# friendlymatthew/heif

Hardware: NVIDIA B200
Metric: decoded MP/s (12MP HEIC grid batch) (higher is better)
Workload: dtype u8

## Files before the change

heif_b200/csrc/cuda/deblock_kernel.cu:

```cuda
#include <cuda_runtime.h>

#include "kernels.h"

namespace heic {
namespace dev {

namespace {

__device__ const uint8_t kBetaTable[52] = {0,  0,  0,  0,  0,  0,  0,  0,  0,  0,  0,  0,  0,  0,  0,  0,  6,  7,
                                           8,  9,  10, 11, 12, 13, 14, 15, 16, 17, 18, 20, 22, 24, 26, 28, 30, 32,
                                           34, 36, 38, 40, 42, 44, 46, 48, 50, 52, 54, 56, 58, 60, 62, 64};
__device__ const uint8_t kTcTable[54] = {0, 0, 0, 0, 0, 0, 0, 0, 0, 0, 0,  0,  0,  0,  0,  0,  0,  0,
                                         1, 1, 1, 1, 1, 1, 1, 1, 1, 2, 2,  2,  2,  3,  3,  3,  3,  4,
                                         4, 4, 5, 5, 6, 6, 7, 8, 9, 10, 11, 13, 14, 16, 18, 20, 22, 24};
__device__ const uint8_t kChromaQp[14] = {29, 30, 31, 32, 33, 33, 34, 34, 35, 35, 36, 36, 37, 37};

__device__ __forceinline__ int clip3(int lo, int hi, int v) { return min(hi, max(lo, v)); }
__device__ __forceinline__ int clip8(int v) { return min(255, max(0, v)); }

__device__ __forceinline__ uint32_t interleave4(uint32_t v) {
  v &= 0x0fu;
  v = (v | (v << 2)) & 0x33u;
  v = (v | (v << 1)) & 0x55u;
  return v;
}

struct Pic {
  const uint32_t* tu_map;
  const uint8_t* qp_map;
  int w8, log2_ctb, wctb;
};

__device__ __forceinline__ bool is_tu_edge(const Pic& p, int x, int y, int pos) {
  const int ctb4 = 1 << (p.log2_ctb - 2);
  const int rx = x >> p.log2_ctb, ry = y >> p.log2_ctb;
  const uint32_t z = interleave4((uint32_t)(x >> 2) & (ctb4 - 1)) | (interleave4((uint32_t)(y >> 2) & (ctb4 - 1)) << 1);
  const uint32_t* tu = p.tu_map + (size_t)(ry * p.wctb + rx) * (ctb4 * ctb4);
  const uint32_t w3 = tu[z & ~63u], w2 = tu[z & ~15u];
  const bool in32 = (w3 & 7u) == (TU_ORIGIN | (3u << 1)) && (pos & 31) != 0;
  const bool in16 = (w2 & 7u) == (TU_ORIGIN | (2u << 1)) && (pos & 15) != 0;
  return !(in32 || in16);
}
__device__ __forceinline__ int qp_at(const Pic& p, int x, int y) { return p.qp_map[(y >> 3) * p.w8 + (x >> 3)]; }

__device__ __forceinline__ int dp4(uint32_t samples, uint32_t weights, int acc) {
  int d;
  asm("dp4a.u32.s32 %0, %1, %2, %3;" : "=r"(d) : "r"(samples), "r"(weights), "r"(acc));
  return d;
}
__host__ __device__ constexpr uint32_t W(int a, int b, int c, int d) {
  return ((uint32_t)a & 0xffu) | (((uint32_t)b & 0xffu) << 8) | (((uint32_t)c & 0xffu) << 16) | (((uint32_t)d & 0xffu) << 24);
}
__device__ __forceinline__ int lin(uint32_t P, uint32_t Q, uint32_t wp, uint32_t wq, int c) { return dp4(Q, wq, dp4(P, wp, c)); }

__device__ __forceinline__ bool filter_luma_segment(uint32_t (&rw)[8][2], int qp_sum, int beta_off2, int tc_off2) {
  const int qpl = (qp_sum + 1) >> 1;
  const int beta = kBetaTable[clip3(0, 51, qpl + beta_off2)];
  const int tc = kTcTable[clip3(0, 53, qpl + 2 + tc_off2)];
  const uint32_t P0 = rw[0][0], Q0 = rw[0][1], P3 = rw[3][0], Q3 = rw[3][1];
  const int dp0 = abs(dp4(P0, W(0, 1, -2, 1), 0)), dp3 = abs(dp4(P3, W(0, 1, -2, 1), 0));
  const int dq0 = abs(dp4(Q0, W(1, -2, 1, 0), 0)), dq3 = abs(dp4(Q3, W(1, -2, 1, 0), 0));
  const int dpq0 = dp0 + dq0, dpq3 = dp3 + dq3, dp = dp0 + dp3, dq = dq0 + dq3;
  if (dpq0 + dpq3 >= beta) return false;
  const int tc25 = (5 * tc + 1) >> 1;
  const bool s0 = 2 * dpq0 < (beta >> 2) && abs(dp4(P0, W(1, 0, 0, -1), 0)) + abs(dp4(Q0, W(1, 0, 0, -1), 0)) < (beta >> 3) &&
                  abs(lin(P0, Q0, W(0, 0, 0, 1), W(-1, 0, 0, 0), 0)) < tc25;
  const bool s3 = 2 * dpq3 < (beta >> 2) && abs(dp4(P3, W(1, 0, 0, -1), 0)) + abs(dp4(Q3, W(1, 0, 0, -1), 0)) < (beta >> 3) &&
                  abs(lin(P3, Q3, W(0, 0, 0, 1), W(-1, 0, 0, 0), 0)) < tc25;
  const bool strong = s0 && s3;
  const bool dep = dp < ((beta + (beta >> 1)) >> 3), deq = dq < ((beta + (beta >> 1)) >> 3);
#pragma unroll
  for (int l = 0; l < 4; l++) {
    const uint32_t P = rw[l][0], Q = rw[l][1];
    if (strong) {
      const int t2 = 2 * tc;
      const int e_p0 = clip3(-t2, t2, lin(P, Q, W(0, 1, 2, 2 - 8), W(2, 1, 0, 0), 4) >> 3);
      const int e_p1 = clip3(-t2, t2, lin(P, Q, W(0, 1, 1 - 4, 1), W(1, 0, 0, 0), 2) >> 2);
      const int e_p2 = clip3(-t2, t2, lin(P, Q, W(2, 3 - 8, 1, 1), W(1, 0, 0, 0), 4) >> 3);
      const int e_q0 = clip3(-t2, t2, lin(P, Q, W(0, 0, 1, 2), W(2 - 8, 2, 1, 0), 4) >> 3);
      const int e_q1 = clip3(-t2, t2, lin(P, Q, W(0, 0, 0, 1), W(1, 1 - 4, 1, 0), 2) >> 2);
      const int e_q2 = clip3(-t2, t2, lin(P, Q, W(0, 0, 0, 1), W(1, 1, 3 - 8, 2), 4) >> 3);
      rw[l][0] = P + (uint32_t)e_p2 * 256u + (uint32_t)e_p1 * 65536u + (uint32_t)e_p0 * 16777216u;
      rw[l][1] = Q + (uint32_t)e_q0 + (uint32_t)e_q1 * 256u + (uint32_t)e_q2 * 65536u;
    } else {
      int delta = lin(P, Q, W(0, 0, 3, -9), W(9, -3, 0, 0), 8) >> 4;
      if (abs(delta) < tc * 10) {
        delta = clip3(-tc, tc, delta);
        const int p0 = dp4(P, W(0, 0, 0, 1), 0), q0 = dp4(Q, W(1, 0, 0, 0), 0);
        const int ep = clip8(p0 + delta) - p0, eq = clip8(q0 - delta) - q0;
        uint32_t addp = (uint32_t)ep * 16777216u, addq = (uint32_t)eq;
        if (dep) {
          const int p1 = dp4(P, W(0, 0, 1, 0), 0);
          const int e = clip3(-(tc >> 1), tc >> 1, (((dp4(P, W(0, 1, 0, 1), 1) >> 1) - p1 + delta) >> 1));
          addp += (uint32_t)(clip8(p1 + e) - p1) * 65536u;
        }
        if (deq) {
          const int q1 = dp4(Q, W(0, 1, 0, 0), 0);
          const int e = clip3(-(tc >> 1), tc >> 1, (((dp4(Q, W(1, 0, 1, 0), 1) >> 1) - q1 - delta) >> 1));
          addq += (uint32_t)(clip8(q1 + e) - q1) * 256u;
        }
        rw[l][0] = P + addp;
        rw[l][1] = Q + addq;
      }
    }
  }
  return true;
}

__device__ __forceinline__ bool filter_chroma_segment(uint32_t (&rw)[8][2], int qp_sum, int c_qp_off, int tc_off2) {
  const int qpi = ((qp_sum + 1) >> 1) + c_qp_off;
  const int qpc = qpi < 30 ? qpi : (qpi >= 43 ? qpi - 6 : kChromaQp[qpi - 30]);
  const int tc = kTcTable[clip3(0, 53, qpc + 2 + tc_off2)];
  if (!tc) return false;
#pragma unroll
  for (int l = 0; l < 4; l++) {
    const uint32_t P = rw[l][0], Q = rw[l][1];
    const int delta = clip3(-tc, tc, lin(P, Q, W(0, 0, 1, -4), W(4, -1, 0, 0), 4) >> 3);
    const int p0 = dp4(P, W(0, 0, 0, 1), 0), q0 = dp4(Q, W(1, 0, 0, 0), 0);
    rw[l][0] = P + (uint32_t)(clip8(p0 + delta) - p0) * 16777216u;
    rw[l][1] = Q + (uint32_t)(clip8(q0 - delta) - q0);
  }
  return true;
}

__device__ __forceinline__ void transpose4(uint32_t a, uint32_t b, uint32_t c, uint32_t d, uint32_t& o0, uint32_t& o1, uint32_t& o2, uint32_t& o3) {
  const uint32_t t0 = __byte_perm(a, b, 0x5140), t1 = __byte_perm(c, d, 0x5140);
  const uint32_t t2 = __byte_perm(a, b, 0x7362), t3 = __byte_perm(c, d, 0x7362);
  o0 = __byte_perm(t0, t1, 0x5410);
  o1 = __byte_perm(t0, t1, 0x7632);
  o2 = __byte_perm(t2, t3, 0x5410);
  o3 = __byte_perm(t2, t3, 0x7632);
}
__device__ __forceinline__ void transpose_cell(uint32_t (&rw)[8][2]) {
  uint32_t t[8][2];
  transpose4(rw[0][0], rw[1][0], rw[2][0], rw[3][0], t[0][0], t[1][0], t[2][0], t[3][0]);
  transpose4(rw[4][0], rw[5][0], rw[6][0], rw[7][0], t[0][1], t[1][1], t[2][1], t[3][1]);
  transpose4(rw[0][1], rw[1][1], rw[2][1], rw[3][1], t[4][0], t[5][0], t[6][0], t[7][0]);
  transpose4(rw[4][1], rw[5][1], rw[6][1], rw[7][1], t[4][1], t[5][1], t[6][1], t[7][1]);
#pragma unroll
  for (int r = 0; r < 8; r++) rw[r][0] = t[r][0], rw[r][1] = t[r][1];
}

template <int CIDX>
__device__ __forceinline__ void deblock_cell(const Pic& pic, uint8_t* plane, int pitch, int pw, int ph, int k, int j,
                                             int beta_off2, int tc_off2, int c_qp_off) {
  constexpr int SUB = CIDX ? 1 : 0;
  const int x0 = 8 * k - 4, y0 = 8 * j - 4;
  const bool has_left = k > 0, has_right = 8 * k < pw, has_top = j > 0, has_bottom = 8 * j < ph;
  uint32_t rw[8][2];
#pragma unroll
  for (int r = 0; r < 8; r++) {
    const bool row_ok = r < 4 ? has_top : has_bottom;
    rw[r][0] = rw[r][1] = 0;
    if (row_ok) {
      const uint8_t* row = plane + (size_t)(y0 + r) * pitch;
      if (has_left) rw[r][0] = *reinterpret_cast<const uint32_t*>(row + x0);
      if (has_right) rw[r][1] = *reinterpret_cast<const uint32_t*>(row + x0 + 4);
    }
  }
  const int xe = (8 * k) << SUB, ye = (8 * j) << SUB;
  uint32_t seg_do = 0, seg_qp = 0;
#pragma unroll
  for (int g = 0; g < 4; g++) {
    const bool vert = g < 2;
    const int half = g & 1;
    bool ok;
    if (vert) ok = has_left && has_right && (half == 0 ? has_top : has_bottom);
    else ok = has_top && has_bottom && (half == 0 ? has_left : has_right);
    if (ok) {
      const int xl = vert ? xe : (x0 + 4 * half) << SUB, yl = vert ? (y0 + 4 * half) << SUB : ye;
      seg_qp |= (uint32_t)(qp_at(pic, xl, yl) + (vert ? qp_at(pic, xl - 1, yl) : qp_at(pic, xl, yl - 1))) << (8 * g);
      seg_do |= (is_tu_edge(pic, xl, yl, vert ? xl : yl) ? 1u : 0u) << g;
    }
  }
  if (!seg_do) return;
  bool changed = false;
#pragma unroll 1
  for (int g = 0; g < 4; g++) {
    if ((seg_do >> g) & 1u) {
      const int qp_sum = (int)((seg_qp >> (8 * g)) & 0xffu);
      changed |= CIDX == 0 ? filter_luma_segment(rw, qp_sum, beta_off2, tc_off2) : filter_chroma_segment(rw, qp_sum, c_qp_off, tc_off2);
    }
#pragma unroll
    for (int r = 0; r < 4; r++) {
      uint32_t t0 = rw[r][0], t1 = rw[r][1];
      rw[r][0] = rw[r + 4][0], rw[r][1] = rw[r + 4][1];
      rw[r + 4][0] = t0, rw[r + 4][1] = t1;
    }
    if (g & 1) transpose_cell(rw);
  }
  if (!changed) return;
#pragma unroll
  for (int r = 0; r < 8; r++) {
    const bool row_ok = r < 4 ? has_top : has_bottom;
    if (!row_ok) continue;
    uint8_t* row = plane + (size_t)(y0 + r) * pitch;
    if (has_left) *reinterpret_cast<uint32_t*>(row + x0) = rw[r][0];
    if (has_right) *reinterpret_cast<uint32_t*>(row + x0 + 4) = rw[r][1];
  }
}

#ifndef HEIC_DEBLOCK_MIN_CTAS
#define HEIC_DEBLOCK_MIN_CTAS 12
#endif
template <int KIND>
__global__ void __launch_bounds__(128, HEIC_DEBLOCK_MIN_CTAS) deblock_kernel(Arenas A, uint32_t blocks_per_tile) {
  const uint32_t tile = blockIdx.x / blocks_per_tile;
  const TileParams* tp = A.tiles + tile;
  const PicParams* pp = A.pics + tp->pic;
  if (A.status[tile].code != 0 || tp->deblock_disabled) return;
  if (KIND == 1 && !pp->chroma) return;
  uint32_t g = (blockIdx.x % blocks_per_tile) * blockDim.x + threadIdx.x;
  const int pw = pp->w >> KIND, ph = pp->h >> KIND;
  const uint32_t cx = (uint32_t)((pw + 7) >> 3) + 1, cy = (uint32_t)((ph + 7) >> 3) + 1;
  int cidx = KIND;
  if (g >= cx * cy) {
    if (KIND == 0) return;
    g -= cx * cy;
    cidx = 2;
    if (g >= cx * cy) return;
  }
  const int k = (int)(g % cx), j = (int)(g / cx);
  if (8 * k - 4 >= pw || 8 * j - 4 >= ph) return;
  Pic pic;
  pic.tu_map = A.tu_map + tp->tu_off;
  pic.qp_map = A.qp_map + tp->map8_off;
  pic.w8 = pp->w8;
  pic.log2_ctb = pp->log2_ctb;
  pic.wctb = pp->wctb;
  const int beta_off2 = tp->beta_offset_div2 * 2, tc_off2 = tp->tc_offset_div2 * 2;
  deblock_cell<KIND>(pic, A.recon + tp->plane_off[cidx], KIND ? pp->pitch_c : pp->pitch_y, pw, ph, k, j, beta_off2, tc_off2,
                     cidx == 0 ? 0 : (cidx == 1 ? pp->pps_cb_qp_offset : pp->pps_cr_qp_offset));
}

}

cudaError_t launch_deblock(const Arenas& A, uint32_t max_w, uint32_t max_h, cudaStream_t stream) {
  if (!A.n_tiles) return cudaSuccess;
  const uint32_t cells_y = (((max_w + 7) >> 3) + 1) * (((max_h + 7) >> 3) + 1);
  const uint32_t cells_c = 2 * ((((max_w >> 1) + 7) >> 3) + 1) * ((((max_h >> 1) + 7) >> 3) + 1);
  const uint32_t by = (cells_y + 127) / 128, bc = (cells_c + 127) / 128;
  deblock_kernel<0><<<A.n_tiles * by, 128, 0, stream>>>(A, by);
  deblock_kernel<1><<<A.n_tiles * bc, 128, 0, stream>>>(A, bc);
  return cudaGetLastError();
}

}
}
```

Measured before the change: 29020.

## Warp-compact luma deblock filtering by strong/normal class through shared staging

Splits the luma segment filter into a decision step and per-line filters. Each segment's lines are staged in shared memory and redistributed across the warp: strong-filter lines are processed first, then normal-filter lines, one line per lane. The aim is to cut divergence between strong and normal paths across lanes. The change also hoists the QP and TU-map lookups so shared corner values are loaded once per cell, and keeps out-of-range luma threads alive so warp ballots stay full. In exchange it adds shared-memory traffic, __syncwarp barriers and ballot overhead for every segment, plus extra work on dead lanes.

```diff
diff --git a/heif_b200/csrc/cuda/deblock_kernel.cu b/heif_b200/csrc/cuda/deblock_kernel.cu
--- a/heif_b200/csrc/cuda/deblock_kernel.cu
+++ b/heif_b200/csrc/cuda/deblock_kernel.cu
@@ -31,15 +31,16 @@
   int w8, log2_ctb, wctb;
 };
 
-__device__ __forceinline__ bool is_tu_edge(const Pic& p, int x, int y, int pos) {
+__device__ __forceinline__ uint32_t tu_units(const Pic& p, int x, int y) {
   const int ctb4 = 1 << (p.log2_ctb - 2);
   const int rx = x >> p.log2_ctb, ry = y >> p.log2_ctb;
   const uint32_t z = interleave4((uint32_t)(x >> 2) & (ctb4 - 1)) | (interleave4((uint32_t)(y >> 2) & (ctb4 - 1)) << 1);
   const uint32_t* tu = p.tu_map + (size_t)(ry * p.wctb + rx) * (ctb4 * ctb4);
   const uint32_t w3 = tu[z & ~63u], w2 = tu[z & ~15u];
-  const bool in32 = (w3 & 7u) == (TU_ORIGIN | (3u << 1)) && (pos & 31) != 0;
-  const bool in16 = (w2 & 7u) == (TU_ORIGIN | (2u << 1)) && (pos & 15) != 0;
-  return !(in32 || in16);
+  return (uint32_t)((w3 & 7u) == (TU_ORIGIN | (3u << 1))) | (uint32_t)((w2 & 7u) == (TU_ORIGIN | (2u << 1))) << 1;
+}
+__device__ __forceinline__ uint32_t is_tu_edge(uint32_t units, int pos) {
+  return !(((units & 1u) && (pos & 31) != 0) || ((units & 2u) && (pos & 15) != 0));
 }
 __device__ __forceinline__ int qp_at(const Pic& p, int x, int y) { return p.qp_map[(y >> 3) * p.w8 + (x >> 3)]; }
 
@@ -53,7 +54,7 @@
 }
 __device__ __forceinline__ int lin(uint32_t P, uint32_t Q, uint32_t wp, uint32_t wq, int c) { return dp4(Q, wq, dp4(P, wp, c)); }
 
-__device__ __forceinline__ bool filter_luma_segment(uint32_t (&rw)[8][2], int qp_sum, int beta_off2, int tc_off2) {
+__device__ __forceinline__ uint32_t decide_luma_segment(const uint32_t (&rw)[8][2], int qp_sum, int beta_off2, int tc_off2) {
   const int qpl = (qp_sum + 1) >> 1;
   const int beta = kBetaTable[clip3(0, 51, qpl + beta_off2)];
   const int tc = kTcTable[clip3(0, 53, qpl + 2 + tc_off2)];
@@ -61,50 +62,84 @@
   const int dp0 = abs(dp4(P0, W(0, 1, -2, 1), 0)), dp3 = abs(dp4(P3, W(0, 1, -2, 1), 0));
   const int dq0 = abs(dp4(Q0, W(1, -2, 1, 0), 0)), dq3 = abs(dp4(Q3, W(1, -2, 1, 0), 0));
   const int dpq0 = dp0 + dq0, dpq3 = dp3 + dq3, dp = dp0 + dp3, dq = dq0 + dq3;
-  if (dpq0 + dpq3 >= beta) return false;
   const int tc25 = (5 * tc + 1) >> 1;
-  const bool s0 = 2 * dpq0 < (beta >> 2) && abs(dp4(P0, W(1, 0, 0, -1), 0)) + abs(dp4(Q0, W(1, 0, 0, -1), 0)) < (beta >> 3) &&
-                  abs(lin(P0, Q0, W(0, 0, 0, 1), W(-1, 0, 0, 0), 0)) < tc25;
-  const bool s3 = 2 * dpq3 < (beta >> 2) && abs(dp4(P3, W(1, 0, 0, -1), 0)) + abs(dp4(Q3, W(1, 0, 0, -1), 0)) < (beta >> 3) &&
-                  abs(lin(P3, Q3, W(0, 0, 0, 1), W(-1, 0, 0, 0), 0)) < tc25;
-  const bool strong = s0 && s3;
+  const bool s0 = (2 * dpq0 < (beta >> 2)) & (abs(dp4(P0, W(1, 0, 0, -1), 0)) + abs(dp4(Q0, W(1, 0, 0, -1), 0)) < (beta >> 3)) &
+                  (abs(lin(P0, Q0, W(0, 0, 0, 1), W(-1, 0, 0, 0), 0)) < tc25);
+  const bool s3 = (2 * dpq3 < (beta >> 2)) & (abs(dp4(P3, W(1, 0, 0, -1), 0)) + abs(dp4(Q3, W(1, 0, 0, -1), 0)) < (beta >> 3)) &
+                  (abs(lin(P3, Q3, W(0, 0, 0, 1), W(-1, 0, 0, 0), 0)) < tc25);
   const bool dep = dp < ((beta + (beta >> 1)) >> 3), deq = dq < ((beta + (beta >> 1)) >> 3);
-#pragma unroll
-  for (int l = 0; l < 4; l++) {
-    const uint32_t P = rw[l][0], Q = rw[l][1];
-    if (strong) {
-      const int t2 = 2 * tc;
-      const int e_p0 = clip3(-t2, t2, lin(P, Q, W(0, 1, 2, 2 - 8), W(2, 1, 0, 0), 4) >> 3);
-      const int e_p1 = clip3(-t2, t2, lin(P, Q, W(0, 1, 1 - 4, 1), W(1, 0, 0, 0), 2) >> 2);
-      const int e_p2 = clip3(-t2, t2, lin(P, Q, W(2, 3 - 8, 1, 1), W(1, 0, 0, 0), 4) >> 3);
-      const int e_q0 = clip3(-t2, t2, lin(P, Q, W(0, 0, 1, 2), W(2 - 8, 2, 1, 0), 4) >> 3);
-      const int e_q1 = clip3(-t2, t2, lin(P, Q, W(0, 0, 0, 1), W(1, 1 - 4, 1, 0), 2) >> 2);
-      const int e_q2 = clip3(-t2, t2, lin(P, Q, W(0, 0, 0, 1), W(1, 1, 3 - 8, 2), 4) >> 3);
-      rw[l][0] = P + (uint32_t)e_p2 * 256u + (uint32_t)e_p1 * 65536u + (uint32_t)e_p0 * 16777216u;
-      rw[l][1] = Q + (uint32_t)e_q0 + (uint32_t)e_q1 * 256u + (uint32_t)e_q2 * 65536u;
-    } else {
-      int delta = lin(P, Q, W(0, 0, 3, -9), W(9, -3, 0, 0), 8) >> 4;
-      if (abs(delta) < tc * 10) {
-        delta = clip3(-tc, tc, delta);
-        const int p0 = dp4(P, W(0, 0, 0, 1), 0), q0 = dp4(Q, W(1, 0, 0, 0), 0);
-        const int ep = clip8(p0 + delta) - p0, eq = clip8(q0 - delta) - q0;
-        uint32_t addp = (uint32_t)ep * 16777216u, addq = (uint32_t)eq;
-        if (dep) {
-          const int p1 = dp4(P, W(0, 0, 1, 0), 0);
-          const int e = clip3(-(tc >> 1), tc >> 1, (((dp4(P, W(0, 1, 0, 1), 1) >> 1) - p1 + delta) >> 1));
-          addp += (uint32_t)(clip8(p1 + e) - p1) * 65536u;
-        }
-        if (deq) {
-          const int q1 = dp4(Q, W(0, 1, 0, 0), 0);
-          const int e = clip3(-(tc >> 1), tc >> 1, (((dp4(Q, W(1, 0, 1, 0), 1) >> 1) - q1 - delta) >> 1));
-          addq += (uint32_t)(clip8(q1 + e) - q1) * 256u;
-        }
-        rw[l][0] = P + addp;
-        rw[l][1] = Q + addq;
-      }
-    }
-  }
-  return true;
+  const uint32_t d = 1u | (uint32_t)(s0 & s3) << 1 | (uint32_t)dep << 2 | (uint32_t)deq << 3 | (uint32_t)tc << 4;
+  return dpq0 + dpq3 < beta ? d : 0u;
+}
+
+__device__ __forceinline__ void strong_luma_line(uint32_t& P, uint32_t& Q, int tc) {
+  const int t2 = 2 * tc;
+  const int e_p0 = clip3(-t2, t2, lin(P, Q, W(0, 1, 2, 2 - 8), W(2, 1, 0, 0), 4) >> 3);
+  const int e_p1 = clip3(-t2, t2, lin(P, Q, W(0, 1, 1 - 4, 1), W(1, 0, 0, 0), 2) >> 2);
+  const int e_p2 = clip3(-t2, t2, lin(P, Q, W(2, 3 - 8, 1, 1), W(1, 0, 0, 0), 4) >> 3);
+  const int e_q0 = clip3(-t2, t2, lin(P, Q, W(0, 0, 1, 2), W(2 - 8, 2, 1, 0), 4) >> 3);
+  const int e_q1 = clip3(-t2, t2, lin(P, Q, W(0, 0, 0, 1), W(1, 1 - 4, 1, 0), 2) >> 2);
+  const int e_q2 = clip3(-t2, t2, lin(P, Q, W(0, 0, 0, 1), W(1, 1, 3 - 8, 2), 4) >> 3);
+  P += (uint32_t)e_p2 * 256u + (uint32_t)e_p1 * 65536u + (uint32_t)e_p0 * 16777216u;
+  Q += (uint32_t)e_q0 + (uint32_t)e_q1 * 256u + (uint32_t)e_q2 * 65536u;
+}
+
+__device__ __forceinline__ void normal_luma_line(uint32_t& P, uint32_t& Q, int tc, bool dep, bool deq) {
+  int delta = lin(P, Q, W(0, 0, 3, -9), W(9, -3, 0, 0), 8) >> 4;
+  const bool on = abs(delta) < tc * 10;
+  delta = clip3(-tc, tc, delta);
+  const int p0 = dp4(P, W(0, 0, 0, 1), 0), q0 = dp4(Q, W(1, 0, 0, 0), 0);
+  const int p1 = dp4(P, W(0, 0, 1, 0), 0), q1 = dp4(Q, W(0, 1, 0, 0), 0);
+  const int ep1 = clip3(-(tc >> 1), tc >> 1, (((dp4(P, W(0, 1, 0, 1), 1) >> 1) - p1 + delta) >> 1));
+  const int eq1 = clip3(-(tc >> 1), tc >> 1, (((dp4(Q, W(1, 0, 1, 0), 1) >> 1) - q1 - delta) >> 1));
+  const uint32_t addp = (uint32_t)(clip8(p0 + delta) - p0) * 16777216u + (dep ? (uint32_t)(clip8(p1 + ep1) - p1) * 65536u : 0u);
+  const uint32_t addq = (uint32_t)(clip8(q0 - delta) - q0) + (deq ? (uint32_t)(clip8(q1 + eq1) - q1) * 256u : 0u);
+  P += on ? addp : 0u;
+  Q += on ? addq : 0u;
+}
+
+struct LumaStage {
+  uint2 line[32 * 4];
+  uint32_t list[32];
+};
+__device__ __forceinline__ int stage_slot(uint32_t seg, uint32_t l) { return (int)(seg * 4 + ((l + (seg >> 2)) & 3)); }
+
+__device__ __forceinline__ void filter_luma_warp(uint32_t (&rw)[8][2], uint32_t d, LumaStage& st) {
+  const uint32_t lane = threadIdx.x & 31;
+  const uint32_t S = __ballot_sync(~0u, (d & 3u) == 3u), N = __ballot_sync(~0u, (d & 3u) == 1u);
+  if (!(S | N)) return;
+  const uint32_t lt = (1u << lane) - 1u;
+  const int nS = __popc(S), nN = __popc(N);
+  if (d) {
+    st.list[(d & 2u) ? __popc(S & lt) : nS + __popc(N & lt)] = lane | d << 5;
+#pragma unroll
+    for (int l = 0; l < 4; l++) st.line[stage_slot(lane, l)] = make_uint2(rw[l][0], rw[l][1]);
+  }
+  __syncwarp();
+#pragma unroll 1
+  for (int t = (int)lane; t < 4 * nS; t += 32) {
+    const uint32_t e = st.list[t >> 2];
+    const int i = stage_slot(e & 31u, (uint32_t)t & 3u);
+    uint2 v = st.line[i];
+    strong_luma_line(v.x, v.y, (int)(e >> 9));
+    st.line[i] = v;
+  }
+#pragma unroll 1
+  for (int t = (int)lane; t < 4 * nN; t += 32) {
+    const uint32_t e = st.list[nS + (t >> 2)];
+    const int i = stage_slot(e & 31u, (uint32_t)t & 3u);
+    uint2 v = st.line[i];
+    normal_luma_line(v.x, v.y, (int)(e >> 9), (e >> 7) & 1u, (e >> 8) & 1u);
+    st.line[i] = v;
+  }
+  __syncwarp();
+  if (d) {
+#pragma unroll
+    for (int l = 0; l < 4; l++) {
+      const uint2 v = st.line[stage_slot(lane, l)];
+      rw[l][0] = v.x, rw[l][1] = v.y;
+    }
+  }
 }
 
 __device__ __forceinline__ bool filter_chroma_segment(uint32_t (&rw)[8][2], int qp_sum, int c_qp_off, int tc_off2) {
@@ -142,11 +177,11 @@
 }
 
 template <int CIDX>
-__device__ __forceinline__ void deblock_cell(const Pic& pic, uint8_t* plane, int pitch, int pw, int ph, int k, int j,
-                                             int beta_off2, int tc_off2, int c_qp_off) {
+__device__ __forceinline__ void deblock_cell(const Pic& pic, uint8_t* plane, int pitch, int pw, int ph, int k, int j, bool live,
+                                             int beta_off2, int tc_off2, int c_qp_off, LumaStage* st) {
   constexpr int SUB = CIDX ? 1 : 0;
   const int x0 = 8 * k - 4, y0 = 8 * j - 4;
-  const bool has_left = k > 0, has_right = 8 * k < pw, has_top = j > 0, has_bottom = 8 * j < ph;
+  const bool has_left = live && k > 0, has_right = live && 8 * k < pw, has_top = live && j > 0, has_bottom = live && 8 * j < ph;
   uint32_t rw[8][2];
 #pragma unroll
   for (int r = 0; r < 8; r++) {
@@ -159,27 +194,27 @@
     }
   }
   const int xe = (8 * k) << SUB, ye = (8 * j) << SUB;
-  uint32_t seg_do = 0, seg_qp = 0;
-#pragma unroll
+  const int s4 = 4 << SUB;
+  const bool v0 = has_left && has_right && has_top, v1 = has_left && has_right && has_bottom;
+  const bool h0 = has_top && has_bottom && has_left, h1 = has_top && has_bottom && has_right;
+  const int q00 = has_top && has_left ? qp_at(pic, xe - 1, ye - 1) : 0, q01 = has_top && has_right ? qp_at(pic, xe, ye - 1) : 0;
+  const int q10 = has_bottom && has_left ? qp_at(pic, xe - 1, ye) : 0, q11 = has_bottom && has_right ? qp_at(pic, xe, ye) : 0;
+  const uint32_t u_top = v0 ? tu_units(pic, xe, ye - s4) : 0u, u_left = h0 ? tu_units(pic, xe - s4, ye) : 0u;
+  const uint32_t u_mid = v1 || h1 ? tu_units(pic, xe, ye) : 0u;
+  const uint32_t seg_do = (uint32_t)(v0 && is_tu_edge(u_top, xe)) | (uint32_t)(v1 && is_tu_edge(u_mid, xe)) << 1 |
+                          (uint32_t)(h0 && is_tu_edge(u_left, ye)) << 2 | (uint32_t)(h1 && is_tu_edge(u_mid, ye)) << 3;
+  const uint32_t seg_qp = (uint32_t)(q00 + q01) | (uint32_t)(q10 + q11) << 8 | (uint32_t)(q00 + q10) << 16 | (uint32_t)(q01 + q11) << 24;
+  if (CIDX == 0 ? !__ballot_sync(~0u, seg_do) : !seg_do) return;
+  bool changed = false;
+#pragma unroll 4
   for (int g = 0; g < 4; g++) {
-    const bool vert = g < 2;
-    const int half = g & 1;
-    bool ok;
-    if (vert) ok = has_left && has_right && (half == 0 ? has_top : has_bottom);
-    else ok = has_top && has_bottom && (half == 0 ? has_left : has_right);
-    if (ok) {
-      const int xl = vert ? xe : (x0 + 4 * half) << SUB, yl = vert ? (y0 + 4 * half) << SUB : ye;
-      seg_qp |= (uint32_t)(qp_at(pic, xl, yl) + (vert ? qp_at(pic, xl - 1, yl) : qp_at(pic, xl, yl - 1))) << (8 * g);
-      seg_do |= (is_tu_edge(pic, xl, yl, vert ? xl : yl) ? 1u : 0u) << g;
-    }
-  }
-  if (!seg_do) return;
-  bool changed = false;
-#pragma unroll 1
-  for (int g = 0; g < 4; g++) {
-    if ((seg_do >> g) & 1u) {
-      const int qp_sum = (int)((seg_qp >> (8 * g)) & 0xffu);
-      changed |= CIDX == 0 ? filter_luma_segment(rw, qp_sum, beta_off2, tc_off2) : filter_chroma_segment(rw, qp_sum, c_qp_off, tc_off2);
+    const int qp_sum = (int)((seg_qp >> (8 * g)) & 0xffu);
+    if (CIDX == 0) {
+      const uint32_t d = decide_luma_segment(rw, qp_sum, beta_off2, tc_off2) & (0u - ((seg_do >> g) & 1u));
+      changed |= d != 0;
+      filter_luma_warp(rw, d, *st);
+    } else if ((seg_do >> g) & 1u) {
+      changed |= filter_chroma_segment(rw, qp_sum, c_qp_off, tc_off2);
     }
 #pragma unroll
     for (int r = 0; r < 4; r++) {
@@ -210,18 +245,21 @@
   const PicParams* pp = A.pics + tp->pic;
   if (A.status[tile].code != 0 || tp->deblock_disabled) return;
   if (KIND == 1 && !pp->chroma) return;
+  __shared__ LumaStage stage[128 / 32];
   uint32_t g = (blockIdx.x % blocks_per_tile) * blockDim.x + threadIdx.x;
   const int pw = pp->w >> KIND, ph = pp->h >> KIND;
   const uint32_t cx = (uint32_t)((pw + 7) >> 3) + 1, cy = (uint32_t)((ph + 7) >> 3) + 1;
   int cidx = KIND;
-  if (g >= cx * cy) {
-    if (KIND == 0) return;
+  bool live = g < cx * cy;
+  if (KIND == 1 && !live) {
     g -= cx * cy;
     cidx = 2;
     if (g >= cx * cy) return;
+    live = true;
   }
   const int k = (int)(g % cx), j = (int)(g / cx);
-  if (8 * k - 4 >= pw || 8 * j - 4 >= ph) return;
+  live = live && 8 * k - 4 < pw && 8 * j - 4 < ph;
+  if (KIND == 1 && !live) return;
   Pic pic;
   pic.tu_map = A.tu_map + tp->tu_off;
   pic.qp_map = A.qp_map + tp->map8_off;
@@ -229,8 +267,9 @@
   pic.log2_ctb = pp->log2_ctb;
   pic.wctb = pp->wctb;
   const int beta_off2 = tp->beta_offset_div2 * 2, tc_off2 = tp->tc_offset_div2 * 2;
-  deblock_cell<KIND>(pic, A.recon + tp->plane_off[cidx], KIND ? pp->pitch_c : pp->pitch_y, pw, ph, k, j, beta_off2, tc_off2,
-                     cidx == 0 ? 0 : (cidx == 1 ? pp->pps_cb_qp_offset : pp->pps_cr_qp_offset));
+  deblock_cell<KIND>(pic, A.recon + tp->plane_off[cidx], KIND ? pp->pitch_c : pp->pitch_y, pw, ph, k, j, live, beta_off2,
+                     tc_off2, cidx == 0 ? 0 : (cidx == 1 ? pp->pps_cb_qp_offset : pp->pps_cr_qp_offset),
+                     KIND == 0 ? &stage[threadIdx.x >> 5] : nullptr);
 }
 
 }
```

Result: no change. 29190 (median of 6 runs) (+0.6%).
